# DRSY/EasyKV

Hardware: AMD Instinct MI355X
Metric: decode_tokens_per_sec (higher is better)
Workload: dtype f16 storage / f32 accumulate; 1 GPU; bench-D decode at fixed budget: B=1 L=32 Hq=32 H=32 D=128 budget=2048 T=2049 kv_policy=roco (Llama2-7B shape, budget=50% of S=4096); parallelism=1 GPU, layers_per_launch=32, layers_per_rank=32, sequences_per_launch=1, n_split=1, fused=True, slot_map=scattered (random permutation: long-run steady state), prewarm_steps=4096, hipgraph=False, overlap_scorer=False, handoff=False

## Files before the change

easykv_amd/_lib.py:

```python
from __future__ import annotations

import ctypes as C
import os

import torch

from ._build import LIB

POLICY_NONE, POLICY_H2O_HEAD, POLICY_ROCO, POLICY_TOVA, POLICY_RANGE = 0, 1, 2, 3, 4
PHASE_SLOT_TAIL_OK = 32
PHASE_SLOT_ROWS = 16
POLICY_CODES = {"full": POLICY_NONE, "h2o_head": POLICY_H2O_HEAD, "roco": POLICY_ROCO, "tova": POLICY_TOVA,
                "recency": POLICY_RANGE, "random": POLICY_RANGE}

DTYPE_F16, DTYPE_BF16 = 0, 1
DTYPE_CODES = {torch.float16: DTYPE_F16, torch.bfloat16: DTYPE_BF16}

MAX_SEQS = 64
DTYPE_F32 = 2
STEP_CALLS = ("step_check", "step_info", "workspace_bytes", "step_attend")


def step_call_name(rows, batch, what):
    if rows is None and not batch:
        return "ekv_" + what + "_typed"
    return "ekv_" + (rows + "_" if rows else "") + ("batch_" if batch else "") + what


EXPORTS = ("ekv_abi_version", "ekv_strerror", "ekv_workspace_bytes", "ekv_step_plan", "ekv_bank_reset", "ekv_state_init",
           "ekv_step_attend", "ekv_gather_ordered", "ekv_scatter_rows", "ekv_compact_inplace", "ekv_step_check", "ekv_step_info",
           "ekv_rows_to_slots", "ekv_rows_to_order", "ekv_kv8_quantize", "ekv_kv8_dequantize", "ekv_kv4_quantize", "ekv_kv4_dequantize",
           "ekv_kv6_quantize", "ekv_kv6_dequantize", "ekv_set_resident_bytes", "ekv_step_resident_rows", "ekv_kv84_quantize", "ekv_kv84_dequantize",
           "ekv_kv164_quantize", "ekv_kv164_dequantize") + tuple(
               step_call_name(rows, batch, what) for rows in (None, "kv8", "kv4", "kv6", "kv84", "kv164") for batch in (False, True) for what in STEP_CALLS)
LONG_CALLS = {what: "ekv_long_" + what for what in STEP_CALLS}
EXPORTS += tuple(LONG_CALLS[what] for what in STEP_CALLS)
LONG_INFO_N = 12
CAP_CALLS = {what: "ekv_cap_" + what for what in STEP_CALLS}
EXPORTS += tuple(CAP_CALLS[what] for what in STEP_CALLS) + ("ekv_softcap_eval",)


class Bank(C.Structure):
    _fields_ = [("k", C.c_void_p), ("v", C.c_void_p), ("slot_of_pos", C.c_void_p),
                ("score_sum", C.c_void_p), ("score_sq", C.c_void_p), ("score_cnt", C.c_void_p),
                ("n_layers", C.c_int32), ("n_q_heads", C.c_int32), ("n_kv_heads", C.c_int32),
                ("head_dim", C.c_int32), ("cap", C.c_int32), ("arrive", C.c_void_p), ("birth", C.c_void_p), ("slot_state", C.c_void_p)]


# ... 56 lines not shown
    lib.ekv_workspace_bytes.restype = C.c_size_t
    lib.ekv_workspace_bytes.argtypes = [C.POINTER(Bank), C.POINTER(Step)]
    lib.ekv_step_plan.argtypes = [C.POINTER(Bank), C.POINTER(Step), C.POINTER(C.c_int32), C.POINTER(C.c_int32)]
    lib.ekv_bank_reset.argtypes = [C.POINTER(Bank), vp]
    lib.ekv_state_init.argtypes = [C.POINTER(Bank), i32, i32, i32, i32, i32, vp]
    lib.ekv_step_attend.argtypes = [C.POINTER(Bank), C.POINTER(Step), vp, vp, vp, vp, vp, vp, vp, vp, C.c_size_t, vp]
    lib.ekv_gather_ordered.argtypes = [C.POINTER(Bank), i32, i32, i32, vp, vp, vp]
    lib.ekv_scatter_rows.argtypes = [C.POINTER(Bank), i32, i32, i32, i32, vp, vp, vp]
    lib.ekv_compact_inplace.argtypes = [C.POINTER(Bank), i32, i32, i32, i32, vp, vp]
    lib.ekv_step_check.argtypes = [C.POINTER(Bank), C.POINTER(Step)]
    lib.ekv_step_info.argtypes = [C.POINTER(Bank), C.POINTER(Step), C.POINTER(C.c_int32), C.c_int32]
    lib.ekv_rows_to_slots.argtypes = [C.POINTER(Bank), i32, i32, i32, vp]
    lib.ekv_rows_to_order.argtypes = [C.POINTER(Bank), i32, i32, i32, vp]
    lib.ekv_set_resident_bytes.argtypes = [C.c_int64]
    lib.ekv_step_resident_rows.argtypes = [C.POINTER(Bank), C.POINTER(Step), i32]
    tails = {"step_check": [], "workspace_bytes": [], "step_info": [C.POINTER(C.c_int32), C.c_int32]}
    for rows, desc in ((None, None), ("kv8", Kv8), ("kv4", Kv4), ("kv6", Kv6), ("kv84", Kv84), ("kv164", Kv164)):
        for batch in (False, True):
            head = [C.POINTER(Bank), C.POINTER(Step), i32] + ([C.POINTER(desc)] if desc else []) + ([C.POINTER(Seq), i32] if batch else [])
            tails["step_attend"] = [vp] * (6 if batch else 8) + [C.c_size_t, vp]
            for what in STEP_CALLS:
                getattr(lib, step_call_name(rows, batch, what)).argtypes = head + tails[what]
        if rows is None:
            tails["step_attend"] = [vp] * 8 + [C.c_size_t, vp]
            for what in STEP_CALLS:
                getattr(lib, LONG_CALLS[what]).argtypes = [C.POINTER(Bank), C.POINTER(Step), i32] + tails[what]
                getattr(lib, CAP_CALLS[what]).argtypes = [C.POINTER(Bank), C.POINTER(Step), i32, C.c_float] + tails[what]
        if desc:
            getattr(lib, f"ekv_{rows}_quantize").argtypes = [C.POINTER(Bank), C.POINTER(desc), i32, i32, i32, i32, vp]
            getattr(lib, f"ekv_{rows}_dequantize").argtypes = [C.POINTER(Bank), C.POINTER(desc), i32, i32, i32, i32, vp, vp, vp]
    lib.ekv_softcap_eval.argtypes = [vp, C.c_int64, C.c_float, C.c_float, vp, vp]
    lib.ekv_kv164_dequantize.argtypes = [C.POINTER(Bank), C.POINTER(Kv164), i32, i32, i32, i32, vp, vp]
    for name in EXPORTS:
        if name != "ekv_strerror":
            getattr(lib, name).restype = C.c_size_t if "workspace_bytes" in name else C.c_int
    if lib.ekv_abi_version() != 8:
        raise EkvError("ABI version mismatch")
    _lib = lib
    return lib


def set_resident_bytes(nbytes):
    load().ekv_set_resident_bytes(-1 if nbytes is None or nbytes < 0 else int(nbytes))


def check(code: int, what: str):
    if code != 0:
        msg = load().ekv_strerror(code).decode()
        if code == -1:
            raise ValueError(f"{what}: {msg}")
        raise EkvError(f"{what}: {msg} ({code})")
```

easykv_amd/csrc/ekv_abi.hip:

```cpp
#include "ekv_common.h"
#include "ekv_kernels.h"
#include "ekv_plan.h"

static inline void drop_stale_error() { (void)hipGetLastError(); }
static inline int launch_code(hipError_t e) { return e == hipSuccess ? EKV_OK : EKV_E_LAUNCH; }

static int call_attend(const EkvCall& c, const void* q, const void* k_new, const void* v_new, void* out, int32_t* evict_ids,
                       const float* rope_cos, const float* rope_sin, void* workspace, size_t workspace_bytes, void* stream) {
  EkvResolved r;
  if (int e = resolve_call(c, &r)) return e;
  const ekv_bank* bank = r.bank;
  const ekv_step* st = r.step;
  const EkvSeqTable* tb = r.tb;
  const EkvStepPlan& P = r.plan;
  if (!q || !k_new || !v_new || !out || !workspace || (st->rope_on_read && (!rope_cos || !rope_sin))) return EKV_E_ARG;
  if (P.bytes > workspace_bytes) return EKV_E_WORKSPACE;
  hipStream_t s = static_cast<hipStream_t>(stream);
  const int n = st->q_len, D = bank->head_dim, lc = st->layer_count;
  char* const ws = static_cast<char*>(workspace);
  auto f32 = [&](int64_t off) { return off < 0 ? nullptr : reinterpret_cast<float*>(ws + off); };
  auto f16 = [&](int64_t off) { return off < 0 ? nullptr : reinterpret_cast<__half*>(ws + off); };

  EkvAttnArgs aa{};
  aa.k = static_cast<const __half*>(bank->k);
// ... 118 lines not shown

int ekv_step_plan(const ekv_bank* bank, const ekv_step* st, int32_t* n_split, int32_t* fused) { return call_plan(bank, st, n_split, fused); }

int ekv_step_info_typed(const ekv_bank* bank, const ekv_step* st, int32_t dtype, int32_t* info, int32_t n_info) {
  return call_info(step_call(bank, st, dtype), info, n_info);
}
int ekv_step_info(const ekv_bank* bank, const ekv_step* st, int32_t* info, int32_t n_info) {
  return call_info(step_call(bank, st, EKV_DTYPE_F16), info, n_info);
}

int ekv_set_resident_bytes(int64_t bytes) {
  ekv_resident_set_budget_bytes(bytes);
  return EKV_OK;
}
int ekv_step_resident_rows(const ekv_bank* bank, const ekv_step* st, int32_t dtype) { return call_resident_rows(step_call(bank, st, dtype)); }

int ekv_step_check_typed(const ekv_bank* bank, const ekv_step* st, int32_t dtype) { return call_check(step_call(bank, st, dtype)); }
int ekv_step_check(const ekv_bank* bank, const ekv_step* st) { return call_check(step_call(bank, st, EKV_DTYPE_F16)); }

int ekv_step_attend(const ekv_bank* bank, const ekv_step* st, const void* q, const void* k_new, const void* v_new,
                    void* out, int32_t* evict_ids, const float* rope_cos, const float* rope_sin, void* workspace,
                    size_t workspace_bytes, void* stream) {
  return call_attend(step_call(bank, st, EKV_DTYPE_F16), q, k_new, v_new, out, evict_ids, rope_cos, rope_sin, workspace, workspace_bytes, stream);
}
int ekv_step_attend_typed(const ekv_bank* bank, const ekv_step* st, int32_t dtype, const void* q, const void* k_new,
                          const void* v_new, void* out, int32_t* evict_ids, const float* rope_cos, const float* rope_sin,
                          void* workspace, size_t workspace_bytes, void* stream) {
  return call_attend(step_call(bank, st, dtype), q, k_new, v_new, out, evict_ids, rope_cos, rope_sin, workspace, workspace_bytes, stream);
}

// ... 359 lines not shown
```

easykv_amd/csrc/ekv_attn_decode.inc:

```
#ifdef EKV_TAIL_PROFILE
#define EKV_STAMP(i) do { if (threadIdx.x == 0) stamps[i] = __builtin_readcyclecounter(); } while (0)
#endif
#include "ekv_decode_stream.h"
#include "ekv_decode_tail.h"
#ifndef EKV_KV8
#define EKV_KV8 0
#endif
#ifndef EKV_BATCH
#define EKV_BATCH 0
#endif
#ifndef EKV_KV4
#define EKV_KV4 0
#endif
#ifndef EKV_KV6
#define EKV_KV6 0
#endif
#if EKV_KV4 || EKV_KV6
#define EKV_MX 1
#else
#define EKV_MX 0
#endif
#ifndef EKV_KV84
#define EKV_KV84 0
#endif
// ... 111 lines not shown
  const int lane = tid & 63, wave = tid >> 6;
  const int T = a.n_slots;
  const int nrep = (REP == 1 || REP == 2) ? REP : a.n_q_heads / a.n_kv_heads;
  const bool roco = sc.policy == EKV_POLICY_ROCO;
  const bool scored = roco || sc.policy == EKV_POLICY_H2O_HEAD || sc.policy == EKV_POLICY_TOVA;
  const int off = scored ? sc.score_off : 0;
  const int W = SLOT ? a.phys_extent : T - off;
  const int w_pad = (int)ekv_align((size_t)W, 256);
#ifdef EKV_NO_PHYS
  constexpr bool PHYS = false;
#else
  constexpr bool PHYS = !ROPE;
#endif
  const int l_pad = a.l_pad;
  constexpr bool kResident = D == 128 && REP == 1 && PHYS && SLOT && !EKV_G8 && !EKV_MX && !EKV_KV164 && !EKV_BATCH;
  const int res_rows = kResident ? EKV_RESIDENT_ROWS(a.fused_order) : 0;
  float* s_logit = reinterpret_cast<float*>(smem);
  float* s_part = s_logit + (size_t)REP * l_pad;
  float* sS = s_part + (size_t)Gm::NP * REP * Gm::PS + ((Gm::NP * REP * Gm::PS) & 3 ? 4 - ((Gm::NP * REP * Gm::PS) & 3) : 0);
  float* sQ = sS + w_pad;
  float* sC = sQ + w_pad;
  RedN<NW> red;
  red.buf = reinterpret_cast<unsigned long long*>(sS + (size_t)(roco ? (SLOT ? 2 : 3) : 1) * w_pad);
  red.phase = 0;
  red.lane = lane;
  red.wave = wave;
  const size_t head_row = ((size_t)(a.layer_begin + ll) * a.n_kv_heads + h) * a.cap;
#ifdef EKV_TAIL_PROFILE
  unsigned long long* stamps = reinterpret_cast<unsigned long long*>(sc.tova_row) + ((size_t)ll * a.n_kv_heads + h) * 8;
#endif
  EKV_STAMP(0);
// ... 24 lines not shown
  if (SLOT) {
    const size_t head = (size_t)(a.layer_begin + ll) * a.n_kv_heads + h;
    g_old = sc.slot_state[4 * head];
    nb = reinterpret_cast<const int32_t*>(sc.slot_state)[4 * head + 1];
    c_new = sc.cnt_tail[head_row + T - 1] - g_old;
  }
  const int E = a.phys_extent;
  const int fl_idx = T - 1 + tid;
  int fl = 0;
  if (PHYS) {
    fl = slot_row[min(fl_idx, a.cap - 1)];
    const int n_words = (int)ekv_align((size_t)E, 128) / 32;
    for (int i = tid; i < n_words; i += 64 * NW)
      s_deadw[i] = i * 32 >= E ? ~0u : (i * 32 + 32 > E ? ~0u << (E & 31) : 0u);
  }
  auto mask_ready = [&]() {
    ekv_lds_barrier();
    if (fl_idx < a.cap && fl < E) atomicOr(&s_deadw[fl >> 5], 1u << (fl & 31));
    for (int i = fl_idx + 64 * NW; i < a.cap; i += 64 * NW) {
      const int row = slot_row[i];
      if (row < E) atomicOr(&s_deadw[row >> 5], 1u << (row & 31));
    }
    ekv_lds_barrier();
  };

  if constexpr (kOrders) {
    if (order_k) {
      constexpr int LPR = Gm::LPR;
      const int sub = lane % LPR, grp = lane / LPR;
      const int new_row = slot_row[T - 1];
// ... 2 lines not shown
      float mk = EKV_NEG_INF;
      ekv_decode_plane_loop<D, NW, kResident>(a.k, head_row, E, mask_ready, [&](uint4 (&kr)[8], const int j0) {
        const unsigned dead8 = (unsigned)s_dead[j0 >> 3];
        float s[8];
#pragma unroll
        for (int u = 0; u < 8; ++u) {
          const float acc = ekv_group_sum<LPR>(ekv_dot8(qv, kr[u], 0.f));
          s[u] = !((dead8 >> u) & 1u) ? EKV_LOGIT(acc, a) : EKV_NEG_INF;
        }
        float mine = s[0];
#pragma unroll
        for (int u = 1; u < 8; ++u) mine = (sub == u) ? s[u] : mine;
        if (sub < 8 && !((dead8 >> sub) & 1u)) s_logit[j0 + sub] = mine;
#pragma unroll
        for (int u = 0; u < 8; ++u) mk = fmaxf(mk, s[u]);
      }, res_rows);
      const __half* v_new_row = a.v_new + ((size_t)ll * a.n_kv_heads + h) * D;
      if (wave == 0 && grp == 0) {
        const uint4 kn = reinterpret_cast<const uint4*>(a.k_new + ((size_t)ll * a.n_kv_heads + h) * D)[sub];
        const uint4 vn = reinterpret_cast<const uint4*>(v_new_row)[sub];
        const size_t off_new = (head_row + new_row) * D;
        reinterpret_cast<uint4*>(a.k_w + off_new)[sub] = kn;
        reinterpret_cast<uint4*>(a.v_w + off_new)[sub] = vn;
        const float acc = EKV_LOGIT(ekv_group_sum<LPR>(ekv_dot8(qv, kn, 0.f)), a);
        if (sub == 0) s_logit[new_row] = acc;
        mk = fmaxf(mk, acc);
      }
      ekv_tail_prefetch_ragged<NW>(sc, head_row, W, roco, sS, sQ, sC, false);
      float cC[ITEMS];
      int32_t cB[ITEMS];
#pragma unroll
// ... 36 lines not shown
#pragma unroll
        for (int u = 1; u < 8; ++u) mx = fmaxf(mx, s[u]);
        const float mn = fmaxf(m[0], mx);
        if (mn == EKV_NEG_INF) return;
        const float alpha = exp2f((m[0] - mn) * EKV_LOG2E);
        l[0] *= alpha;
#pragma unroll
        for (int i = 0; i < 8; ++i) o[0][i] *= alpha;
#pragma unroll
        for (int u = 0; u < 8; ++u) {
          const float p = exp2f((s[u] - mn) * EKV_LOG2E);
          l[0] += p;
          ekv_axpy8(p, vr[u], o[0]);
        }
        m[0] = mn;
      }, res_rows);
      if (wave == 0 && grp == 0) {
        const uint4 vn = reinterpret_cast<const uint4*>(v_new_row)[sub];
        const float acc = s_logit[new_row];
        const float mn = fmaxf(m[0], acc);
        const float alpha = m[0] == EKV_NEG_INF ? 0.f : exp2f((m[0] - mn) * EKV_LOG2E);
        const float p = exp2f((acc - mn) * EKV_LOG2E);
        l[0] = l[0] * alpha + p;
#pragma unroll
        for (int i = 0; i < 8; ++i) o[0][i] *= alpha;
        ekv_axpy8(p, vn, o[0]);
        m[0] = mn;
      }
      ekv_decode_wave_combine<D, 1>(m, l, o);
      ekv_decode_stash<D, 1, NW>(s_part, m, l, o);
      __syncthreads();
// ... 6 lines not shown
#ifdef EKV_TAIL_PROFILE
      if (tid == 0) {
        stamps[3] = 1;
        stamps[6] = __builtin_amdgcn_s_getreg(63492);
        stamps[7] = __builtin_amdgcn_s_getreg(63508);
      }
#endif
      return;
    }
  }

  constexpr int KUF = ROPE ? EKV_ROPE_KU(REP) : (EKV_KV164 && REP == 1 ? EKV_KV164_FUSED_KU1 : EKV_FUSED_KU);
  float m[REP], l[REP], o[REP][kEPL];
  if (PHYS)
    ekv_decode_stream<D, REP, ROPE, false, NW, PHYS, KUF, decltype(mask_ready), kEPL, kFMT, kResident>(a, slot_row, s_logit, l_pad, 0, T, ll, h, head_row, m, l, o,
                                                     reinterpret_cast<const uint8_t*>(s_deadw), mask_ready, nrep, h * nrep, res_rows);
  else
    ekv_decode_stream<D, REP, ROPE, false, NW, false, KUF, EkvNoop, kEPL, kFMT>(a, slot_row, s_logit, l_pad, 0, T, ll, h, head_row, m, l, o, nullptr,
                                                      EkvNoop(), nrep, h * nrep);
  if (scored) ekv_tail_prefetch_ragged<NW>(sc, head_row, W, roco, sS, sQ, sC, !SLOT);
  float cC[SLOT ? ITEMS : 1];
  int32_t cB[SLOT ? ITEMS : 1];
  if (SLOT) {
#pragma unroll
    for (int it = 0; it < (SLOT ? ITEMS : 1); ++it) {
      const int j = min(tid + it * 64 * NW, a.cap - 1);
      cC[it] = roco ? sc.score_cnt[head_row + j] : 0.f;
      cB[it] = sc.birth[head_row + j];
    }
  }

// ... 118 lines not shown
```

easykv_amd/csrc/ekv_decode_stream.h:

```cpp
#pragma once
#include "ekv_common.h"
#include "ekv_kernels.h"


struct EkvNoop {
  __device__ __forceinline__ void operator()() const {}
};
#ifndef EKV_ROPE_MOCK
#define EKV_ROPE_MOCK 0
#endif
template <bool RESIDENT>
__device__ __forceinline__ uint4 ekv_load_row_piece(const char* row, int sub) {
  const ekv_u4* p = reinterpret_cast<const ekv_u4*>(row) + sub;
  if constexpr (RESIDENT) return __builtin_bit_cast(uint4, *p);
  else return __builtin_bit_cast(uint4, __builtin_nontemporal_load(p));
}
template <bool B>
struct EkvBool {
  static constexpr bool value = B;
};

template <int D, int REP, bool ROPE, bool SLOT_LDS, int NW = 4, bool PHYS = false, int KU = kU, typename MaskReady = EkvNoop, int EPL = 8, int FMT = 0, bool RES = false>
__device__ __forceinline__ void ekv_decode_stream(const EkvAttnArgs& a, const int32_t* s_slot, float* logit_out,
                                                  int logit_stride, int t0, int t1_in, int ll, int h, size_t head_row,
                                                  float (&m)[REP], float (&l)[REP], float (&o)[REP][EPL],
                                                  const uint8_t* s_dead = nullptr, MaskReady mask_ready = MaskReady(),
                                                  int n_rep_real = 0, int q_head0 = -1, int res_rows = 0) {
  static_assert(!RES || (PHYS && EPL == 8 && D == 128), "resident rows: 16-bit rows of head_dim 128 (whole lane groups) in physical order");
  using Gm = EkvDecodeGeom<D, NW, KU, EPL>;
  constexpr int LPR = Gm::LPR, RW = Gm::RW, LIVE = Gm::LIVE;
  constexpr bool KV8 = EPL == 16, KV4 = EPL == 32;
  constexpr bool KV6 = KV4 && FMT == 6;
  constexpr bool KV84 = KV8 && FMT == 84;
  constexpr bool KV164 = EPL == 8 && FMT == 164;
  constexpr bool V4 = KV84 || KV164;
  constexpr int VSH = KV164 ? 2 : 1;
  static_assert(FMT == 0 || KV6 || KV84 || KV164,
                "format tag: 6 = MXFP6 rows (EPL = 32), 84 = FP8 keys with MXFP4 values (EPL = 16), 164 = 16-bit keys with MXFP4 values (EPL = 8)");
  static_assert(!KV84 || (D == 128 && LPR == 8), "FP8-key / MXFP4-value rows: head_dim 128 (a lane pair = one 32-element V block)");
  static_assert(!KV164 || (D == 128 && LPR == 16 && !ROPE && !RES), "16-bit-key / MXFP4-value rows: plain keys, head_dim 128 (a lane quad = one 32-element V block), no resident rows");
  static_assert(EPL == 8 || (KV8 && !ROPE && LIVE == LPR) || KV4, "FP8 rows: plain keys, head_dim 64 / 128");
  static_assert(!KV4 || (!ROPE && D == 128 && LPR == 4), "MXFP4 rows: plain keys, head_dim 128 (a lane = one 32-element block)");
  constexpr int ESZ = KV8 ? 1 : 2;
  constexpr int ROWB = KV6 ? 3 * D / 4 : (KV4 ? D / 2 : D * ESZ);
// ... 226 lines not shown
    appended_row();
    return;
  }

  if (PHYS) t1 = a.phys_extent;
  const int last_slot = PHYS ? 0 : s_slot[t1 - 1 - slot_base];
  const int idx_cap = (a.cap - KU) & ~(KU - 1);
  uint4 iv[KU / 4];
#pragma unroll
  for (int i = 0; i < KU / 4; ++i) iv[i] = uint4{0, 0, 0, 0};
  if (!PHYS && !SLOT_LDS && t0 + wave * RW < t1) {
    const uint4* ip = reinterpret_cast<const uint4*>(s_slot + min(t0 + wave * RW + grp * KU, idx_cap));
#pragma unroll
    for (int i = 0; i < KU / 4; ++i) iv[i] = ip[i];
  }
  auto iteration = [&](const int base, auto&& after_issue) {
    uint4 kr[KU], vr[KU];
    ekv_u6 kr6[KV6 ? KU : 1], vr6[KV6 ? KU : 1];
    float ksc[KV8 || KV4 ? KU : 1], vsc[KV8 || KV4 || KV164 ? KU : 1];
    const int j0 = base + grp * KU;
    if constexpr (KV8 && PHYS) {
      if (j0 + KU <= a.cap) {
        const float4* k4 = reinterpret_cast<const float4*>(a.k_scale + head_row + j0);
        const float4* v4 = reinterpret_cast<const float4*>(a.v_scale + head_row + j0);
#pragma unroll
        for (int i = 0; i < KU / 4; ++i) {
          const float4 kk = k4[i], vv = KV84 ? float4{1.f, 1.f, 1.f, 1.f} : v4[i];
          ksc[4 * i] = kk.x, ksc[4 * i + 1] = kk.y, ksc[4 * i + 2] = kk.z, ksc[4 * i + 3] = kk.w;
          vsc[4 * i] = vv.x, vsc[4 * i + 1] = vv.y, vsc[4 * i + 2] = vv.z, vsc[4 * i + 3] = vv.w;
        }
      } else {
// ... 56 lines not shown
      const uint4* ip = reinterpret_cast<const uint4*>(s_slot + min(j0 + kNW * RW, idx_cap));
#pragma unroll
      for (int i = 0; i < KU / 4; ++i) iv[i] = ip[i];
    }
    if constexpr (RES) {
      auto request = [&](auto resident) {
        int jr = j0;
        asm volatile("" : "+v"(jr));
#pragma unroll
        for (int u = 0; u < KU; ++u) {
          const int row = jr + u < t1 ? jr + u : t1 - 1;
          kr[u] = ekv_load_row_piece<decltype(resident)::value>(reinterpret_cast<const char*>(a.k) + (head_row + row) * ROWB, sub);
          vr[u] = ekv_load_row_piece<decltype(resident)::value>(reinterpret_cast<const char*>(a.v) + (head_row + row) * ROWB, sub);
        }
      };
      if (base < res_rows) request(EkvBool<true>());
      else request(EkvBool<false>());
    } else {
#pragma unroll
    for (int u = 0; u < KU; ++u) {
      const int j = j0 + u;
      const int jj = j < t1 ? j : t1 - 1;
      const int row = PHYS ? jj : (SLOT_LDS ? s_slot[jj - t0] : (j < t1 ? cur[u] : last_slot));
      const char* kp = reinterpret_cast<const char*>(a.k) + (head_row + row) * ROWB;
      const char* vp = reinterpret_cast<const char*>(a.v) + (head_row + row) * VROWB;
      if constexpr (KV8 && !PHYS) {
        ksc[u] = a.k_scale[head_row + row];
        if constexpr (KV84) vsc[u] = ekv_fp4_exp_scale(a.v_exp[(head_row + row) * 4 + (sub >> 1)]);
        else vsc[u] = a.v_scale[head_row + row];
      }
      if constexpr (KV4 && !PHYS) {
// ... 92 lines not shown
#pragma unroll
      for (int u = 0; u < KU; ++u) {
        const float p = exp2f((s[u] - mn) * EKV_LOG2E);
        l[r] += p;
        if constexpr (KV84) ekv_axpy16_fp4(p, vsc[u], uint2{vr[u].x, vr[u].y}, o[r]);
        else if constexpr (KV8) ekv_axpy16_fp8(p * vsc[u], vr[u], o[r]);
        else if constexpr (KV6) ekv_axpy32_fp6(p, vsc[u], vr6[u], o[r]);
        else if constexpr (KV4) ekv_axpy32_fp4(p, vsc[u], vr[u], o[r]);
        else if constexpr (KV164) ekv_axpy8_fp4(p, vsc[u], vr[u].x, o[r]);
        else ekv_axpy8(p, vr[u], o[r]);
      }
      m[r] = mn;
    }
  };
  int base = t0 + wave * RW;
  if (PHYS) {
    if (t1 > (kNW - 1) * RW) {
      iteration(base, mask_ready);
      base += kNW * RW;
    } else {
      mask_ready();
    }
  }
  for (; base < t1; base += kNW * RW) iteration(base, EkvNoop());
  appended_row();
}

template <int D, int REP, int EPL = 8>
__device__ __forceinline__ void ekv_decode_wave_combine(float (&m)[REP], float (&l)[REP], float (&o)[REP][EPL]) {
  using Gm = EkvDecodeGeom<D, 4, kU, EPL>;
#pragma unroll
  for (int off = Gm::LPR; off < 64; off <<= 1) {
#pragma unroll
    for (int r = 0; r < REP; ++r) {
      const float mo = __shfl_xor(m[r], off, 64), lo = __shfl_xor(l[r], off, 64);
      const float mn = fmaxf(m[r], mo);
      const float wa = (m[r] == EKV_NEG_INF) ? 0.f : exp2f((m[r] - mn) * EKV_LOG2E);
      const float wb = (mo == EKV_NEG_INF) ? 0.f : exp2f((mo - mn) * EKV_LOG2E);
      l[r] = l[r] * wa + lo * wb;
// ... 29 lines not shown
  mm = EKV_NEG_INF;
#pragma unroll
  for (int i = 0; i < Gm::NP; ++i) mm = fmaxf(mm, s_part[((size_t)i * REP + r) * Gm::PS]);
  ls = 0.f;
  os = 0.f;
#pragma unroll
  for (int i = 0; i < Gm::NP; ++i) {
    const float* p = s_part + ((size_t)i * REP + r) * Gm::PS;
    const float w = (p[0] == EKV_NEG_INF) ? 0.f : exp2f((p[0] - mm) * EKV_LOG2E);
    ls += p[1] * w;
    os += p[2 + d] * w;
  }
}

template <int D, int NW, bool RES = false, typename First, typename Consume>
__device__ __forceinline__ void ekv_decode_plane_loop(const __half* plane, size_t head_row, int t1, First&& first, Consume&& consume, int res_rows = 0) {
  using Gm = EkvDecodeGeom<D, NW, 8, 8>;
  static_assert(Gm::LIVE == Gm::LPR, "whole lane groups");
  constexpr int RW = Gm::RW, STEP = NW * RW;
  const int lane = threadIdx.x & 63, wave = threadIdx.x >> 6;
  const int sub = lane % Gm::LPR, grp = lane / Gm::LPR;
  auto request_as = [&](auto resident, uint4 (&r)[8], int base) {
    int j0 = base + grp * 8;
    if constexpr (RES) asm volatile("" : "+v"(j0));
#pragma unroll
    for (int u = 0; u < 8; ++u) {
      const int row = j0 + u < t1 ? j0 + u : t1 - 1;
      const char* p = reinterpret_cast<const char*>(plane) + (head_row + row) * (D * 2);
      r[u] = ekv_load_row_piece<decltype(resident)::value>(p, sub);
    }
  };
  auto request = [&](uint4 (&r)[8], int base) {
    if constexpr (RES) {
      if (min(base, t1 - 1) < res_rows) request_as(EkvBool<true>(), r, base);
      else request_as(EkvBool<false>(), r, base);
    } else {
      request_as(EkvBool<false>(), r, base);
    }
  };
  uint4 ra[8], rb[8];
  int base = wave * RW;
  request(ra, base);
  first();
  while (base < t1) {
    request(rb, base + STEP);
    consume(ra, base + grp * 8);
    base += STEP;
    if (base >= t1) break;
    request(ra, base + STEP);
// ... 5 lines not shown
```

easykv_amd/csrc/ekv_geometry.h:

```cpp
#pragma once
#include <stddef.h>
#include <stdint.h>

#include "../../include/easykv_hip.h"

#if defined(__HIP__)
#define EKV_HD __host__ __device__
#else
#define EKV_HD
#endif

static inline EKV_HD size_t ekv_align(size_t x, size_t a) { return (x + a - 1) / a * a; }

constexpr int kU = 8;

template <int D, int NW = 4, int KU = kU, int EPL = 8>
struct EkvDecodeGeom {
  static constexpr int LIVE = D / EPL;
  static constexpr int LPR = LIVE <= 4 ? 4 : (LIVE <= 8 ? 8 : (LIVE <= 16 ? 16 : 32));
  static constexpr int G = 64 / LPR;
  static constexpr int RW = G * KU;
  static constexpr int NP = NW;
  static constexpr int PS = D + 2;
  static_assert(D % EPL == 0 && LIVE >= 1, "a row is a whole number of 16-byte pieces");
// ... 4 lines not shown
template <int D, int REP, int NW = 8>
inline size_t ekv_fused_lds(int t_pad, int l_pad, int n_state) {
  using Gm = EkvDecodeGeom<D, NW>;
  const size_t part = ekv_align((size_t)Gm::NP * REP * Gm::PS, 4);
  return ((size_t)REP * l_pad + part + (size_t)n_state * ekv_align((size_t)t_pad, 256)) * 4 + 2 * NW * 8 * 8 +
         ekv_align(ekv_align((size_t)l_pad, 128) / 8, 16) + 264 * 4;
}
template <int D>
inline size_t ekv_fused_lds_max(int rep, int t_pad, int l_pad, int nw) {
  switch (rep) {
    case 1: return nw == 8 ? ekv_fused_lds<D, 1, 8>(t_pad, l_pad, 3) : ekv_fused_lds<D, 1, 4>(t_pad, l_pad, 3);
    case 2: return nw == 8 ? ekv_fused_lds<D, 2, 8>(t_pad, l_pad, 3) : ekv_fused_lds<D, 2, 4>(t_pad, l_pad, 3);
    case 3: case 4: return nw == 8 ? ekv_fused_lds<D, 4, 8>(t_pad, l_pad, 3) : ekv_fused_lds<D, 4, 4>(t_pad, l_pad, 3);
    default: return nw == 8 ? ekv_fused_lds<D, 8, 8>(t_pad, l_pad, 3) : ekv_fused_lds<D, 8, 4>(t_pad, l_pad, 3);
  }
}

#ifndef EKV_SCORE_NW
#define EKV_SCORE_NW 8
#endif
constexpr int kSNW = EKV_SCORE_NW, kSNT = 64 * kSNW;

inline size_t ekv_decode_score_lds(int rep, int t_pad, int policy) {
  const size_t n_state = policy == EKV_POLICY_ROCO ? 3 : 1;
  return ((size_t)rep * t_pad + n_state * ekv_align((size_t)t_pad, 256)) * 4 + 2 * kSNW * 8 * 8 + 264 * 4 + kSNT * 8;
}

inline size_t ekv_score_lds_bytes(int nt, int64_t W, int64_t rows, bool big) {
  return ekv_align(((size_t)(big ? 1 : 4) * (size_t)W + 2 * (size_t)rows) * 4, 16) + 2 * (nt / 64) * 8 * 4 + 264 * 4 + nt * 8;
}
// ... 117 lines not shown
```

easykv_amd/csrc/ekv_kernels.h:

```cpp
#pragma once
#include <hip/hip_runtime.h>
#include <hip/hip_fp16.h>
#include <stdint.h>

#include "../../include/easykv_hip.h"
#include "ekv_geometry.h"

enum EkvRows : int32_t { EKV_ROWS_kv16, EKV_ROWS_kv8, EKV_ROWS_kv4, EKV_ROWS_kv6, EKV_ROWS_kv84, EKV_ROWS_kv164 };

#define EKV_RESIDENT_UNIT 32
#define EKV_RESIDENT_BITS(rows) ((((rows) / EKV_RESIDENT_UNIT) > 255 ? 255 : ((rows) / EKV_RESIDENT_UNIT)) << 16)
#define EKV_RESIDENT_ROWS(order) ((((order) >> 16) & 255) * EKV_RESIDENT_UNIT)

enum EkvLaunchKind : int32_t {
  EKV_RUN_FUSED_DECODE,
  EKV_RUN_CHUNK_LDS,
  EKV_RUN_RESIDENT,
  EKV_RUN_DECODE,
  EKV_RUN_CHUNK,
  EKV_RUN_FLUSH,
  EKV_RUN_FOLD, EKV_RUN_RANGE, EKV_RUN_DECODE_SCORE, EKV_RUN_TOVA_MEAN, EKV_RUN_SCORE_SELECT,
  EKV_RUN_LONG_FOLD,
  EKV_RUN_LONG_SCORE
};
struct EkvLaunch {
  int32_t kind, kernel_count;
  int32_t skip_fold;
// ... 263 lines not shown
```

easykv_amd/csrc/ekv_plan.cpp:

```cpp
#include "ekv_plan.h"

#include <algorithm>
#include <cstdio>
#include <cstdlib>

namespace {

typedef int64_t i64;

bool env_is_1(const char* name) { const char* e = std::getenv(name); return e != nullptr && e[0] == '1'; }
int env_int(const char* name, int otherwise) { const char* e = std::getenv(name); return e != nullptr ? std::atoi(e) : otherwise; }

bool pow2_to_16(int rep) { return rep == 1 || rep == 2 || rep == 4 || rep == 8 || rep == 16; }

}

int check_bank(const ekv_bank* b) {
  if (!b || !b->k || !b->v || !b->slot_of_pos) return EKV_E_ARG;
  if (b->n_layers <= 0 || b->n_kv_heads <= 0 || b->n_q_heads % b->n_kv_heads || b->cap <= 0) return EKV_E_ARG;
  if (b->head_dim != 32 && b->head_dim != 64 && b->head_dim != 96 && b->head_dim != 128 && b->head_dim != 256) return EKV_E_UNSUPPORTED;
  return EKV_OK;
}

int check_layers(const ekv_bank* b, int begin, int count) {
// ... 42 lines not shown
}
void ekv_resident_set_budget_bytes(i64 bytes) { g_resident_bytes = bytes; }

int ekv_decode_resident_rows(i64 n_heads_in_launch, i64 row_bytes, int phys_extent, int cap, int score_rows, i64 budget_bytes) {
  static const int force = env_int("EKV_RESIDENT_ROWS", -1);
  if (n_heads_in_launch <= 0 || row_bytes <= 0 || phys_extent <= 0 || cap <= 0 || score_rows < 0) return 0;
  const i64 unit = EKV_RESIDENT_UNIT;
  const i64 ext = std::min<i64>(((i64)phys_extent + unit - 1) / unit * unit, 255 * unit);
  if (budget_bytes <= 0) return 0;
  if (force >= 0) return (int)std::min<i64>(force / unit * unit, ext);
  const i64 heads = std::min<i64>(n_heads_in_launch, 1 << 20);
  const i64 score = heads * 4 * cap * (score_rows + 2);
  const i64 per_unit = heads * 2 * unit * std::min<i64>(row_bytes, 1 << 16);
  if (budget_bytes < score) return 0;
  return (int)(std::min<i64>((budget_bytes - score) / per_unit, ext / unit) * unit);
}

bool ekv_decode_fused_supported(int head_dim, int rep, int n_slots, int t_pad, int l_pad, int n_evict, int cap, int nw) {
  if (!ekv_attn_decode_supported(head_dim, rep) || rep > 8 || n_evict > 1 || n_slots > 256 * 24 || (cap & 3) != 0 || cap < 16) return false;
  size_t lds = 1 << 30;
  switch (head_dim) {
    case 32: lds = ekv_fused_lds_max<32>(rep, t_pad, l_pad, nw); break;
    case 64: lds = ekv_fused_lds_max<64>(rep, t_pad, l_pad, nw); break;
    case 96: lds = ekv_fused_lds_max<96>(rep, t_pad, l_pad, nw); break;
    case 128: lds = ekv_fused_lds_max<128>(rep, t_pad, l_pad, nw); break;
    case 256: lds = ekv_fused_lds_max<256>(rep, t_pad, l_pad, nw); break;
  }
  return lds <= (size_t)(nw == 8 ? 150 : 80) * 1024;
}

// ... 254 lines not shown
bool plan_whole_step(const StepShape& s, EkvStepPlan* P, int* rc) {
  const ekv_bank* bank = s.bank;
  const ekv_step* st = &s.st;
  const i64 heads_now = (i64)st->layer_count * bank->n_kv_heads;
  *rc = EKV_OK;
  if (s.n == 1 && st->phases == 0 && P->n_split == 1 &&
      ekv_decode_fused_supported(s.D, s.rep, s.T, P->t_pad, P->l_pad, st->n_evict, bank->cap, P->fused_nw)) {
    if (s.slot_rows && !ekv_slot_rows_supported(bank, st, P->phys_extent, P->t_pad)) {
      *rc = EKV_E_UNSUPPORTED;
      return true;
    }
    P->slot_rows = s.slot_rows ? 1 : 0;
    P->slot_tail_ok = s.slot_rows && s.slot_tail_ok ? 1 : 0;
    P->one_launch = 1;
    P->fused_order = ekv_decode_fused_order(s.D, s.rep, s.scored, s.slot_rows, P->fused_nw, heads_now, P->phys_extent);
    if (s.D == 128 && s.rep == 1 && s.slot_rows && !st->rope_on_read)
      P->fused_order |= EKV_RESIDENT_BITS(ekv_decode_resident_rows(heads_now, 2 * s.D, P->phys_extent, bank->cap,
                                                                   st->policy == EKV_POLICY_ROCO ? 3 : 1, ekv_resident_budget_bytes()));
    run(P, EKV_RUN_FUSED_DECODE, 1);
    return true;
  }
  if (s.slot_rows) {
    *rc = EKV_E_UNSUPPORTED;
    return true;
  }
  if (s.n > 1 && !s.capped && ekv_chunk_lds_supported(bank, st, P->phys_extent, s.scored) && (heads_now >= 256 || s.T <= 1024)) {
    P->one_launch = 1;
    run(P, EKV_RUN_CHUNK_LDS, 1);
    return true;
  }
  return false;
}

// ... 292 lines not shown
    if (n_info > 11) info[11] = ok ? P.long_tiles : 0;
  }
  return EKV_OK;
}

int call_resident_rows(const EkvCall& c) {
  EkvResolved r;
  const bool ok = resolve_call(c, &r) == EKV_OK;
  if (c.dtype != EKV_DTYPE_F16 && c.dtype != EKV_DTYPE_BF16) return EKV_E_ARG;
  if (c.rows != EKV_ROWS_kv16 && !r.bank) return EKV_E_ARG;
  if (int e = check_bank(r.bank)) return e;
  if (!c.step || (c.batch && !c.seqs)) return EKV_E_ARG;
  return ok && r.plan.one_launch ? EKV_RESIDENT_ROWS(r.plan.fused_order) : 0;
}

int call_plan(const ekv_bank* bank, const ekv_step* st, int32_t* n_split, int32_t* fused) {
  if (int e = check_bank(bank)) return e;
  if (!st || !n_split || !fused) return EKV_E_ARG;
  EkvResolved r;
  const int rc = resolve_call(step_call(bank, st, EKV_DTYPE_F16), &r);
  *n_split = r.plan.n_split;
  *fused = rc == EKV_OK ? r.plan.one_launch : 0;
  return EKV_OK;
}
```

easykv_amd/csrc/ekv_plan.h:

```cpp
#pragma once
#include "ekv_kernels.h"

int check_bank(const ekv_bank* b);
int check_layers(const ekv_bank* b, int begin, int count);

bool ekv_attn_decode_supported(int head_dim, int rep);
int ekv_decode_fused_nw(int64_t n_heads_in_launch);
int ekv_decode_fused_order(int head_dim, int rep, bool scored, bool slot_rows, int nw, int64_t n_heads_in_launch, int phys_extent);
int ekv_decode_resident_rows(int64_t n_heads_in_launch, int64_t row_bytes, int phys_extent, int cap, int score_rows, int64_t budget_bytes);
int64_t ekv_resident_budget_bytes();
void ekv_resident_set_budget_bytes(int64_t bytes);
bool ekv_decode_fused_supported(int head_dim, int rep, int n_slots, int t_pad, int l_pad, int n_evict, int cap, int nw);
bool ekv_decode_score_supported(const EkvScoreArgs& sc);
bool ekv_attn_chunk_supported(int head_dim, int rep, int q_len);
bool ekv_chunk_two_pass(int head_dim, int rep, int q_len, int policy, bool scored, bool accumulate, bool rope, int mode);
bool ekv_chunk_wide(int head_dim, int rep, int q_len, bool rope, bool two_pass, bool wants_logits);
bool ekv_wide_tail_supported(int64_t W, int64_t n_wg);
bool ekv_attn_resident_supported(int head_dim, int rep, int q_len, int n_slots, int64_t W);
bool ekv_chunk_lds_supported(const ekv_bank* bank, const ekv_step* st, int phys_extent, bool scored);
int ekv_attn_chunk_launches(bool wide, bool rope, bool two_pass, int passes);

EkvScoreArgs score_args(const ekv_bank* bank, const ekv_step* st, const EkvStepPlan& P);
int ekv_plan_step(const ekv_bank* bank, const ekv_step* step, EkvStepPlan* P, bool long_rows = false, bool capped = false);

// ... 62 lines not shown

struct EkvResolved {
  const ekv_bank* bank;
  const ekv_step* step;
  const EkvSeqTable* tb;
  EkvStepPlan plan;
  ekv_bank bank_q;
  ekv_step env;
  EkvSeqTable table;
};
int resolve_call(const EkvCall& c, EkvResolved* r);
int call_check(const EkvCall& c);
size_t call_workspace_bytes(const EkvCall& c);
int call_info(const EkvCall& c, int32_t* info, int32_t n_info);
int call_resident_rows(const EkvCall& c);
int call_plan(const ekv_bank* bank, const ekv_step* st, int32_t* n_split, int32_t* fused);
```

easykv_amd/engine.py:

```python
from __future__ import annotations

import ctypes as C
import math
from dataclasses import dataclass
from typing import Optional

import torch

from . import _lib
from ._lib import Bank, Step, check

DECODE_RECENT_RATIO = 0.3
ROCO_TAIL = 10


@dataclass
class StepPlan:
    policy: str = "roco"
    phase: str = "decode"
    accumulate: bool = True
    evict: bool = False
    score_off: int = 0
    budget: int = 0
    recent: int = 0
# ... 482 lines not shown
        keys = ("n_split", "fused", "two_pass", "wide", "n_qblocks", "qb_rows", "n_col_parts", "fold_in_kernel", "n_launches", "fused_order",
                "long_scorer", "long_tiles")
        return dict(zip(keys, (int(x) for x in info)))

    def resident_rows(self, plan: StepPlan, q_len=1, layer_begin=0, layer_count=None, phases=0) -> int:
        if self._fmt is not None:
            return 0
        st = self.make_step(plan, q_len, layer_begin, self.n_layers - layer_begin if layer_count is None else layer_count)
        st.phases = phases
        _lib.set_resident_bytes(self.resident_bytes)
        rows = self.lib.ekv_step_resident_rows(C.byref(self._bank), C.byref(st), self._dt)
        if rows < 0:
            check(rows, "ekv_step_resident_rows")
        return rows

    def join(self):
        cur = torch.cuda.current_stream(self.device)
        for l, ev in enumerate(self._score_done):
            if ev is not None:
                cur.wait_event(ev)
                self._score_done[l] = None
        self._ws_free = [None] * len(self._ws_free)

    def _attend_overlapped(self, st, q, k_new, v_new, out, evict_ids, lc, layer_begin):
        if self._side is None:
            self._side = [torch.cuda.Stream(self.device) for _ in range(4)]
        main = torch.cuda.current_stream(self.device)
        need = self._step_ws_bytes(st)
        if not self._ws_ring or self._ws_ring[0].numel() < need:
            self._ws_ring = [torch.empty(int(need * 1.25) + 4096, dtype=torch.uint8, device=self.device) for _ in range(8)]
# ... 326 lines not shown
```

include/easykv_hip.h:

```cpp
#ifndef EASYKV_HIP_H
#define EASYKV_HIP_H

#include <stddef.h>
#include <stdint.h>

#ifdef __cplusplus
extern "C" {
#endif

#define EKV_ABI_VERSION 8

enum {
  EKV_POLICY_NONE = 0,
  EKV_POLICY_H2O_HEAD = 1,
  EKV_POLICY_ROCO = 2,
  EKV_POLICY_TOVA = 3,
  EKV_POLICY_RANGE = 4
};

enum {
  EKV_OK = 0,
  EKV_E_ARG = -1,
  EKV_E_UNSUPPORTED = -2,
  EKV_E_WORKSPACE = -3,
// ... 42 lines not shown
  int32_t out_token_stride, out_head_stride;
} ekv_step;

int ekv_abi_version(void);
const char *ekv_strerror(int code);

size_t ekv_workspace_bytes(const ekv_bank *bank, const ekv_step *step);
size_t ekv_workspace_bytes_typed(const ekv_bank *bank, const ekv_step *step, int32_t dtype);

int ekv_step_plan(const ekv_bank *bank, const ekv_step *step, int32_t *n_split, int32_t *fused);

#define EKV_STEP_INFO_N 10
int ekv_step_info(const ekv_bank *bank, const ekv_step *step, int32_t *info, int32_t n_info);
int ekv_step_info_typed(const ekv_bank *bank, const ekv_step *step, int32_t dtype, int32_t *info, int32_t n_info);

int ekv_set_resident_bytes(int64_t bytes);
int ekv_step_resident_rows(const ekv_bank *bank, const ekv_step *step, int32_t dtype);

int ekv_bank_reset(const ekv_bank *bank, void *stream);

int ekv_state_init(const ekv_bank *bank, int32_t layer_begin, int32_t layer_count, int32_t width, int32_t mode,
                   int32_t stride, void *stream);

int ekv_step_attend(const ekv_bank *bank, const ekv_step *step, const void *q, const void *k_new, const void *v_new,
                    void *out, int32_t *evict_ids, const float *rope_cos, const float *rope_sin, void *workspace,
                    size_t workspace_bytes, void *stream);
int ekv_step_attend_typed(const ekv_bank *bank, const ekv_step *step, int32_t dtype, const void *q, const void *k_new,
                          const void *v_new, void *out, int32_t *evict_ids, const float *rope_cos, const float *rope_sin,
                          void *workspace, size_t workspace_bytes, void *stream);

int ekv_step_check(const ekv_bank *bank, const ekv_step *step);
int ekv_step_check_typed(const ekv_bank *bank, const ekv_step *step, int32_t dtype);
// ... 187 lines not shown
```

Baseline: 5942 tokens/s.

## Select resident KV row blocks per wave via bitmask with front/spread layouts

Replaces the scalar resident-row threshold in the fused decode stream with a per-wave 64-bit mask that marks which iterations load rows through the resident (cache-kept) path. A new 'spread' layout distributes resident blocks evenly across each wave's iterations rather than only the front rows, selectable by environment variable. The default stays 'front', so the default behaviour should roughly match the old threshold apart from the mask computation and a new guard that disables residency when extent exceeds 64 iterations per wave. The change adds a ballot and some integer arithmetic per block and exposes query APIs.

```diff
diff --git a/easykv_amd/_lib.py b/easykv_amd/_lib.py
--- a/easykv_amd/_lib.py
+++ b/easykv_amd/_lib.py
@@ -31,7 +31,7 @@
            "ekv_step_attend", "ekv_gather_ordered", "ekv_scatter_rows", "ekv_compact_inplace", "ekv_step_check", "ekv_step_info",
            "ekv_rows_to_slots", "ekv_rows_to_order", "ekv_kv8_quantize", "ekv_kv8_dequantize", "ekv_kv4_quantize", "ekv_kv4_dequantize",
            "ekv_kv6_quantize", "ekv_kv6_dequantize", "ekv_set_resident_bytes", "ekv_step_resident_rows", "ekv_kv84_quantize", "ekv_kv84_dequantize",
-           "ekv_kv164_quantize", "ekv_kv164_dequantize") + tuple(
+           "ekv_kv164_quantize", "ekv_kv164_dequantize", "ekv_step_resident_layout", "ekv_resident_wave_mask") + tuple(
                step_call_name(rows, batch, what) for rows in (None, "kv8", "kv4", "kv6", "kv84", "kv164") for batch in (False, True) for what in STEP_CALLS)
 LONG_CALLS = {what: "ekv_long_" + what for what in STEP_CALLS}
 EXPORTS += tuple(LONG_CALLS[what] for what in STEP_CALLS)
@@ -118,6 +118,8 @@
     lib.ekv_rows_to_order.argtypes = [C.POINTER(Bank), i32, i32, i32, vp]
     lib.ekv_set_resident_bytes.argtypes = [C.c_int64]
     lib.ekv_step_resident_rows.argtypes = [C.POINTER(Bank), C.POINTER(Step), i32]
+    lib.ekv_step_resident_layout.argtypes = [C.POINTER(Bank), C.POINTER(Step), i32]
+    lib.ekv_resident_wave_mask.argtypes = [i32, i32, i32, i32, i32]
     tails = {"step_check": [], "workspace_bytes": [], "step_info": [C.POINTER(C.c_int32), C.c_int32]}
     for rows, desc in ((None, None), ("kv8", Kv8), ("kv4", Kv4), ("kv6", Kv6), ("kv84", Kv84), ("kv164", Kv164)):
         for batch in (False, True):
@@ -138,10 +140,14 @@
     for name in EXPORTS:
         if name != "ekv_strerror":
             getattr(lib, name).restype = C.c_size_t if "workspace_bytes" in name else C.c_int
+    lib.ekv_resident_wave_mask.restype = C.c_uint64
     if lib.ekv_abi_version() != 8:
         raise EkvError("ABI version mismatch")
     _lib = lib
     return lib
+
+
+RESIDENT_LAYOUTS = ("front", "spread")
 
 
 def set_resident_bytes(nbytes):
diff --git a/easykv_amd/csrc/ekv_abi.hip b/easykv_amd/csrc/ekv_abi.hip
--- a/easykv_amd/csrc/ekv_abi.hip
+++ b/easykv_amd/csrc/ekv_abi.hip
@@ -156,6 +156,7 @@
   return EKV_OK;
 }
 int ekv_step_resident_rows(const ekv_bank* bank, const ekv_step* st, int32_t dtype) { return call_resident_rows(step_call(bank, st, dtype)); }
+int ekv_step_resident_layout(const ekv_bank* bank, const ekv_step* st, int32_t dtype) { return call_resident_layout(step_call(bank, st, dtype)); }
 
 int ekv_step_check_typed(const ekv_bank* bank, const ekv_step* st, int32_t dtype) { return call_check(step_call(bank, st, dtype)); }
 int ekv_step_check(const ekv_bank* bank, const ekv_step* st) { return call_check(step_call(bank, st, EKV_DTYPE_F16)); }
diff --git a/easykv_amd/csrc/ekv_attn_decode.inc b/easykv_amd/csrc/ekv_attn_decode.inc
--- a/easykv_amd/csrc/ekv_attn_decode.inc
+++ b/easykv_amd/csrc/ekv_attn_decode.inc
@@ -149,7 +149,6 @@
 #endif
   const int l_pad = a.l_pad;
   constexpr bool kResident = D == 128 && REP == 1 && PHYS && SLOT && !EKV_G8 && !EKV_MX && !EKV_KV164 && !EKV_BATCH;
-  const int res_rows = kResident ? EKV_RESIDENT_ROWS(a.fused_order) : 0;
   float* s_logit = reinterpret_cast<float*>(smem);
   float* s_part = s_logit + (size_t)REP * l_pad;
   float* sS = s_part + (size_t)Gm::NP * REP * Gm::PS + ((Gm::NP * REP * Gm::PS) & 3 ? 4 - ((Gm::NP * REP * Gm::PS) & 3) : 0);
@@ -204,6 +203,8 @@
     for (int i = tid; i < n_words; i += 64 * NW)
       s_deadw[i] = i * 32 >= E ? ~0u : (i * 32 + 32 > E ? ~0u << (E & 31) : 0u);
   }
+  uint64_t res_mask = 0;
+  if constexpr (kResident) res_mask = ekv_resident_wave_bits<NW>(a.fused_order, E, order_k);
   auto mask_ready = [&]() {
     ekv_lds_barrier();
     if (fl_idx < a.cap && fl < E) atomicOr(&s_deadw[fl >> 5], 1u << (fl & 31));
@@ -236,7 +237,7 @@
         if (sub < 8 && !((dead8 >> sub) & 1u)) s_logit[j0 + sub] = mine;
 #pragma unroll
         for (int u = 0; u < 8; ++u) mk = fmaxf(mk, s[u]);
-      }, res_rows);
+      }, res_mask);
       const __half* v_new_row = a.v_new + ((size_t)ll * a.n_kv_heads + h) * D;
       if (wave == 0 && grp == 0) {
         const uint4 kn = reinterpret_cast<const uint4*>(a.k_new + ((size_t)ll * a.n_kv_heads + h) * D)[sub];
@@ -303,7 +304,7 @@
           ekv_axpy8(p, vr[u], o[0]);
         }
         m[0] = mn;
-      }, res_rows);
+      }, res_mask);
       if (wave == 0 && grp == 0) {
         const uint4 vn = reinterpret_cast<const uint4*>(v_new_row)[sub];
         const float acc = s_logit[new_row];
@@ -340,7 +341,7 @@
   float m[REP], l[REP], o[REP][kEPL];
   if (PHYS)
     ekv_decode_stream<D, REP, ROPE, false, NW, PHYS, KUF, decltype(mask_ready), kEPL, kFMT, kResident>(a, slot_row, s_logit, l_pad, 0, T, ll, h, head_row, m, l, o,
-                                                     reinterpret_cast<const uint8_t*>(s_deadw), mask_ready, nrep, h * nrep, res_rows);
+                                                     reinterpret_cast<const uint8_t*>(s_deadw), mask_ready, nrep, h * nrep, res_mask);
   else
     ekv_decode_stream<D, REP, ROPE, false, NW, false, KUF, EkvNoop, kEPL, kFMT>(a, slot_row, s_logit, l_pad, 0, T, ll, h, head_row, m, l, o, nullptr,
                                                       EkvNoop(), nrep, h * nrep);
diff --git a/easykv_amd/csrc/ekv_decode_stream.h b/easykv_amd/csrc/ekv_decode_stream.h
--- a/easykv_amd/csrc/ekv_decode_stream.h
+++ b/easykv_amd/csrc/ekv_decode_stream.h
@@ -9,6 +9,20 @@
 #ifndef EKV_ROPE_MOCK
 #define EKV_ROPE_MOCK 0
 #endif
+template <int NW>
+__device__ __forceinline__ uint64_t ekv_resident_wave_bits(int order, int E, bool plane) {
+  const int r = EKV_RESIDENT_ROWS(order) / EKV_RESIDENT_UNIT;
+  unsigned t = threadIdx.x;
+  asm volatile("" : "+v"(t));
+  const int lane = (int)(t & 63u), wave = __builtin_amdgcn_readfirstlane((int)(t >> 6));
+  const int n = (E + EKV_RESIDENT_UNIT - 1) / EKV_RESIDENT_UNIT, layout = EKV_RESIDENT_LAYOUT(order);
+  const EkvResidentWave p = ekv_resident_wave(layout, n, r, NW, wave);
+  const uint64_t bits = __ballot(ekv_resident_iter(p, lane));
+  if (!plane) return bits;
+  const int nl = n > 0 ? n - 1 : 0;
+  const bool last = ekv_resident_iter(ekv_resident_wave(layout, n, r, NW, nl % NW), nl / NW);
+  return bits | (last && p.n_w < 64 ? ~0ull << (p.n_w & 63) : 0ull);
+}
 template <bool RESIDENT>
 __device__ __forceinline__ uint4 ekv_load_row_piece(const char* row, int sub) {
   const ekv_u4* p = reinterpret_cast<const ekv_u4*>(row) + sub;
@@ -25,9 +39,10 @@
                                                   int logit_stride, int t0, int t1_in, int ll, int h, size_t head_row,
                                                   float (&m)[REP], float (&l)[REP], float (&o)[REP][EPL],
                                                   const uint8_t* s_dead = nullptr, MaskReady mask_ready = MaskReady(),
-                                                  int n_rep_real = 0, int q_head0 = -1, int res_rows = 0) {
+                                                  int n_rep_real = 0, int q_head0 = -1, uint64_t res_mask = 0) {
   static_assert(!RES || (PHYS && EPL == 8 && D == 128), "resident rows: 16-bit rows of head_dim 128 (whole lane groups) in physical order");
   using Gm = EkvDecodeGeom<D, NW, KU, EPL>;
+  static_assert(!RES || Gm::RW == EKV_RESIDENT_UNIT, "resident rows: a wave iteration is one block of the resident layout (ekv_geometry.h)");
   constexpr int LPR = Gm::LPR, RW = Gm::RW, LIVE = Gm::LIVE;
   constexpr bool KV8 = EPL == 16, KV4 = EPL == 32;
   constexpr bool KV6 = KV4 && FMT == 6;
@@ -284,7 +299,7 @@
 #pragma unroll
     for (int i = 0; i < KU / 4; ++i) iv[i] = ip[i];
   }
-  auto iteration = [&](const int base, auto&& after_issue) {
+  auto iteration = [&](const int base, auto&& after_issue, const bool resident) {
     uint4 kr[KU], vr[KU];
     ekv_u6 kr6[KV6 ? KU : 1], vr6[KV6 ? KU : 1];
     float ksc[KV8 || KV4 ? KU : 1], vsc[KV8 || KV4 || KV164 ? KU : 1];
@@ -371,7 +386,7 @@
           vr[u] = ekv_load_row_piece<decltype(resident)::value>(reinterpret_cast<const char*>(a.v) + (head_row + row) * ROWB, sub);
         }
       };
-      if (base < res_rows) request(EkvBool<true>());
+      if (resident) request(EkvBool<true>());
       else request(EkvBool<false>());
     } else {
 #pragma unroll
@@ -494,15 +509,17 @@
     }
   };
   int base = t0 + wave * RW;
+  uint64_t rm = RES ? res_mask : 0;
   if (PHYS) {
     if (t1 > (kNW - 1) * RW) {
-      iteration(base, mask_ready);
+      iteration(base, mask_ready, (rm & 1) != 0);
       base += kNW * RW;
+      rm >>= 1;
     } else {
       mask_ready();
     }
   }
-  for (; base < t1; base += kNW * RW) iteration(base, EkvNoop());
+  for (; base < t1; base += kNW * RW, rm >>= 1) iteration(base, EkvNoop(), (rm & 1) != 0);
   appended_row();
 }
 
@@ -562,7 +579,7 @@
 }
 
 template <int D, int NW, bool RES = false, typename First, typename Consume>
-__device__ __forceinline__ void ekv_decode_plane_loop(const __half* plane, size_t head_row, int t1, First&& first, Consume&& consume, int res_rows = 0) {
+__device__ __forceinline__ void ekv_decode_plane_loop(const __half* plane, size_t head_row, int t1, First&& first, Consume&& consume, uint64_t res_mask = 0) {
   using Gm = EkvDecodeGeom<D, NW, 8, 8>;
   static_assert(Gm::LIVE == Gm::LPR, "whole lane groups");
   constexpr int RW = Gm::RW, STEP = NW * RW;
@@ -578,9 +595,12 @@
       r[u] = ekv_load_row_piece<decltype(resident)::value>(p, sub);
     }
   };
+  uint64_t rm = RES ? res_mask : 0;
   auto request = [&](uint4 (&r)[8], int base) {
     if constexpr (RES) {
-      if (min(base, t1 - 1) < res_rows) request_as(EkvBool<true>(), r, base);
+      const bool resident = (rm & 1) != 0;
+      rm >>= 1;
+      if (resident) request_as(EkvBool<true>(), r, base);
       else request_as(EkvBool<false>(), r, base);
     } else {
       request_as(EkvBool<false>(), r, base);
diff --git a/easykv_amd/csrc/ekv_geometry.h b/easykv_amd/csrc/ekv_geometry.h
--- a/easykv_amd/csrc/ekv_geometry.h
+++ b/easykv_amd/csrc/ekv_geometry.h
@@ -42,6 +42,42 @@
     case 3: case 4: return nw == 8 ? ekv_fused_lds<D, 4, 8>(t_pad, l_pad, 3) : ekv_fused_lds<D, 4, 4>(t_pad, l_pad, 3);
     default: return nw == 8 ? ekv_fused_lds<D, 8, 8>(t_pad, l_pad, 3) : ekv_fused_lds<D, 8, 4>(t_pad, l_pad, 3);
   }
+}
+
+#define EKV_RESIDENT_UNIT 32
+#define EKV_RESIDENT_BITS(rows) ((((rows) / EKV_RESIDENT_UNIT) > 255 ? 255 : ((rows) / EKV_RESIDENT_UNIT)) << 16)
+#define EKV_RESIDENT_ROWS(order) ((((order) >> 16) & 255) * EKV_RESIDENT_UNIT)
+#ifndef EKV_RESIDENT_LAYOUT_DEFAULT
+#define EKV_RESIDENT_LAYOUT_DEFAULT EKV_RESIDENT_LAYOUT_FRONT
+#endif
+#define EKV_RESIDENT_LAYOUT_BIT (1 << 24)
+#define EKV_RESIDENT_LAYOUT_BITS(layout) ((layout) != EKV_RESIDENT_LAYOUT_DEFAULT ? EKV_RESIDENT_LAYOUT_BIT : 0)
+#define EKV_RESIDENT_LAYOUT(order) ((((order) >> 24) & 1) ^ EKV_RESIDENT_LAYOUT_DEFAULT)
+
+struct EkvResidentWave {
+  int layout, n_w, r_w, o_w;
+};
+EKV_HD inline EkvResidentWave ekv_resident_wave(int layout, int n, int r, int nw, int w) {
+  r = r < 0 ? 0 : (r > n ? n : r);
+  EkvResidentWave p;
+  p.layout = layout;
+  p.n_w = n > w ? (n - w + nw - 1) / nw : 0;
+  p.r_w = r / nw + (w < r % nw ? 1 : 0);
+  p.o_w = (w * p.n_w) / nw;
+  return p;
+}
+EKV_HD inline bool ekv_resident_iter(const EkvResidentWave& p, int k) {
+  const unsigned n_w = p.n_w > 0 ? (unsigned)p.n_w : 1u;
+  const bool front = k < p.r_w;
+  const unsigned x = (unsigned)k * (unsigned)p.r_w + (unsigned)p.o_w;
+  const bool spread = x % n_w + (unsigned)p.r_w >= n_w;
+  return (k >= 0) & (k < p.n_w) & (p.layout == EKV_RESIDENT_LAYOUT_FRONT ? front : spread);
+}
+EKV_HD inline uint64_t ekv_resident_mask(int layout, int n, int r, int nw, int w) {
+  const EkvResidentWave p = ekv_resident_wave(layout, n, r, nw, w);
+  uint64_t m = 0;
+  for (int k = 0; k < p.n_w && k < 64; ++k) m |= (uint64_t)(ekv_resident_iter(p, k) ? 1 : 0) << k;
+  return m;
 }
 
 #ifndef EKV_SCORE_NW
diff --git a/easykv_amd/csrc/ekv_kernels.h b/easykv_amd/csrc/ekv_kernels.h
--- a/easykv_amd/csrc/ekv_kernels.h
+++ b/easykv_amd/csrc/ekv_kernels.h
@@ -8,9 +8,6 @@
 
 enum EkvRows : int32_t { EKV_ROWS_kv16, EKV_ROWS_kv8, EKV_ROWS_kv4, EKV_ROWS_kv6, EKV_ROWS_kv84, EKV_ROWS_kv164 };
 
-#define EKV_RESIDENT_UNIT 32
-#define EKV_RESIDENT_BITS(rows) ((((rows) / EKV_RESIDENT_UNIT) > 255 ? 255 : ((rows) / EKV_RESIDENT_UNIT)) << 16)
-#define EKV_RESIDENT_ROWS(order) ((((order) >> 16) & 255) * EKV_RESIDENT_UNIT)
 
 enum EkvLaunchKind : int32_t {
   EKV_RUN_FUSED_DECODE,
diff --git a/easykv_amd/csrc/ekv_plan.cpp b/easykv_amd/csrc/ekv_plan.cpp
--- a/easykv_amd/csrc/ekv_plan.cpp
+++ b/easykv_amd/csrc/ekv_plan.cpp
@@ -3,6 +3,7 @@
 #include <algorithm>
 #include <cstdio>
 #include <cstdlib>
+#include <cstring>
 
 namespace {
 
@@ -80,6 +81,21 @@
   const i64 per_unit = heads * 2 * unit * std::min<i64>(row_bytes, 1 << 16);
   if (budget_bytes < score) return 0;
   return (int)(std::min<i64>((budget_bytes - score) / per_unit, ext / unit) * unit);
+}
+
+int ekv_decode_resident_layout() {
+  static const int layout = [] {
+    const char* e = std::getenv("EKV_RESIDENT_LAYOUT");
+    if (e != nullptr && std::strcmp(e, "front") == 0) return EKV_RESIDENT_LAYOUT_FRONT;
+    if (e != nullptr && std::strcmp(e, "spread") == 0) return EKV_RESIDENT_LAYOUT_SPREAD;
+    return EKV_RESIDENT_LAYOUT_DEFAULT;
+  }();
+  return layout;
+}
+
+extern "C" uint64_t ekv_resident_wave_mask(int32_t n_blocks, int32_t r_blocks, int32_t nw, int32_t wave, int32_t layout) {
+  if (nw < 1 || nw > 64 || wave < 0 || wave >= nw || n_blocks < 0 || n_blocks > (1 << 20) || (layout != EKV_RESIDENT_LAYOUT_FRONT && layout != EKV_RESIDENT_LAYOUT_SPREAD)) return 0;
+  return ekv_resident_mask(layout, n_blocks, r_blocks, nw, wave);
 }
 
 bool ekv_decode_fused_supported(int head_dim, int rep, int n_slots, int t_pad, int l_pad, int n_evict, int cap, int nw) {
@@ -364,9 +380,11 @@
     P->slot_tail_ok = s.slot_rows && s.slot_tail_ok ? 1 : 0;
     P->one_launch = 1;
     P->fused_order = ekv_decode_fused_order(s.D, s.rep, s.scored, s.slot_rows, P->fused_nw, heads_now, P->phys_extent);
-    if (s.D == 128 && s.rep == 1 && s.slot_rows && !st->rope_on_read)
-      P->fused_order |= EKV_RESIDENT_BITS(ekv_decode_resident_rows(heads_now, 2 * s.D, P->phys_extent, bank->cap,
-                                                                   st->policy == EKV_POLICY_ROCO ? 3 : 1, ekv_resident_budget_bytes()));
+    if (s.D == 128 && s.rep == 1 && s.slot_rows && !st->rope_on_read) {
+      int rows = ekv_decode_resident_rows(heads_now, 2 * s.D, P->phys_extent, bank->cap, st->policy == EKV_POLICY_ROCO ? 3 : 1, ekv_resident_budget_bytes());
+      if (((i64)P->phys_extent + EKV_RESIDENT_UNIT - 1) / EKV_RESIDENT_UNIT > 64 * (i64)P->fused_nw) rows = 0;
+      P->fused_order |= EKV_RESIDENT_BITS(rows) | (rows > 0 ? EKV_RESIDENT_LAYOUT_BITS(ekv_decode_resident_layout()) : 0);
+    }
     run(P, EKV_RUN_FUSED_DECODE, 1);
     return true;
   }
@@ -689,6 +707,14 @@
   return ok && r.plan.one_launch ? EKV_RESIDENT_ROWS(r.plan.fused_order) : 0;
 }
 
+int call_resident_layout(const EkvCall& c) {
+  const int rows = call_resident_rows(c);
+  if (rows <= 0) return rows < 0 ? rows : EKV_RESIDENT_LAYOUT_FRONT;
+  EkvResolved r;
+  (void)resolve_call(c, &r);
+  return EKV_RESIDENT_LAYOUT(r.plan.fused_order);
+}
+
 int call_plan(const ekv_bank* bank, const ekv_step* st, int32_t* n_split, int32_t* fused) {
   if (int e = check_bank(bank)) return e;
   if (!st || !n_split || !fused) return EKV_E_ARG;
diff --git a/easykv_amd/csrc/ekv_plan.h b/easykv_amd/csrc/ekv_plan.h
--- a/easykv_amd/csrc/ekv_plan.h
+++ b/easykv_amd/csrc/ekv_plan.h
@@ -8,6 +8,7 @@
 int ekv_decode_fused_nw(int64_t n_heads_in_launch);
 int ekv_decode_fused_order(int head_dim, int rep, bool scored, bool slot_rows, int nw, int64_t n_heads_in_launch, int phys_extent);
 int ekv_decode_resident_rows(int64_t n_heads_in_launch, int64_t row_bytes, int phys_extent, int cap, int score_rows, int64_t budget_bytes);
+int ekv_decode_resident_layout();
 int64_t ekv_resident_budget_bytes();
 void ekv_resident_set_budget_bytes(int64_t bytes);
 bool ekv_decode_fused_supported(int head_dim, int rep, int n_slots, int t_pad, int l_pad, int n_evict, int cap, int nw);
@@ -100,4 +101,5 @@
 size_t call_workspace_bytes(const EkvCall& c);
 int call_info(const EkvCall& c, int32_t* info, int32_t n_info);
 int call_resident_rows(const EkvCall& c);
+int call_resident_layout(const EkvCall& c);
 int call_plan(const ekv_bank* bank, const ekv_step* st, int32_t* n_split, int32_t* fused);
diff --git a/easykv_amd/engine.py b/easykv_amd/engine.py
--- a/easykv_amd/engine.py
+++ b/easykv_amd/engine.py
@@ -520,6 +520,17 @@
             check(rows, "ekv_step_resident_rows")
         return rows
 
+    def resident_layout(self, plan: StepPlan, q_len=1, layer_begin=0, layer_count=None, phases=0) -> str:
+        if self._fmt is not None:
+            return "front"
+        st = self.make_step(plan, q_len, layer_begin, self.n_layers - layer_begin if layer_count is None else layer_count)
+        st.phases = phases
+        _lib.set_resident_bytes(self.resident_bytes)
+        layout = self.lib.ekv_step_resident_layout(C.byref(self._bank), C.byref(st), self._dt)
+        if layout < 0:
+            check(layout, "ekv_step_resident_layout")
+        return _lib.RESIDENT_LAYOUTS[layout]
+
     def join(self):
         cur = torch.cuda.current_stream(self.device)
         for l, ev in enumerate(self._score_done):
diff --git a/include/easykv_hip.h b/include/easykv_hip.h
--- a/include/easykv_hip.h
+++ b/include/easykv_hip.h
@@ -80,8 +80,12 @@
 int ekv_step_info(const ekv_bank *bank, const ekv_step *step, int32_t *info, int32_t n_info);
 int ekv_step_info_typed(const ekv_bank *bank, const ekv_step *step, int32_t dtype, int32_t *info, int32_t n_info);
 
+#define EKV_RESIDENT_LAYOUT_FRONT 0
+#define EKV_RESIDENT_LAYOUT_SPREAD 1
 int ekv_set_resident_bytes(int64_t bytes);
 int ekv_step_resident_rows(const ekv_bank *bank, const ekv_step *step, int32_t dtype);
+int ekv_step_resident_layout(const ekv_bank *bank, const ekv_step *step, int32_t dtype);
+uint64_t ekv_resident_wave_mask(int32_t n_blocks, int32_t r_blocks, int32_t nw, int32_t wave, int32_t layout);
 
 int ekv_bank_reset(const ekv_bank *bank, void *stream);
 
```

New measurement: 5940 tokens/s, median of 2. Within noise of the previous version (-0.0%).
